# cswaney/NetworkHawkesProcesses.jl

Measured on AMD Instinct MI355X. Metric: log-likelihood evals/sec (N=1024, M=1e6), higher is better.
Workload: dtype f64; 1 GPU; continuous exponential standard Hawkes, N=1024, M=1000000, dt_max=1, windowed_k8 (S-metric, SURVEY 8d); pairs_per_eval=7999107, independent_streams=1

## Files before the change

networkhawkesprocesses.jl_amd/csrc/cont_slices.hip:

```cpp
#include <algorithm>
#include <vector>

#include "nhp_internal.h"
#include "nhp_math.h"
#include "nhp_rng.h"

struct nhp_slices {
    const uint32_t *row;
    const int32_t *item0;
    const uint32_t *lo;
    const uint16_t *hi;
    int32_t nsh;
    uint32_t dmask;
    int32_t dbits;
};

#define NHP_SL_SHARDS 64

#ifdef NHP_STAMP
__device__ unsigned long long g_sl_stamps[8 * 4096];
__device__ unsigned long long g_sl_wave_end[16 * 4096];
#define NHP_SL_STAMP(i) do { if (threadIdx.x == 0 && blockIdx.x < 4096) g_sl_stamps[8 * blockIdx.x + (i)] = __builtin_amdgcn_s_memrealtime(); } while (0)
#define NHP_SL_STAMP_WAVE() do { if ((threadIdx.x & 63) == 0 && blockIdx.x < 4096) g_sl_wave_end[16 * blockIdx.x + (threadIdx.x >> 6)] = __builtin_amdgcn_s_memrealtime(); } while (0)
extern "C" int nhp_debug_stamps_slices(unsigned long long *out, int n)
{
    return (int)hipMemcpyFromSymbol(out, HIP_SYMBOL(g_sl_stamps), sizeof(unsigned long long) * (size_t)n);
}
extern "C" int nhp_debug_stamps_slices_waves(unsigned long long *out, int n)
{
    return (int)hipMemcpyFromSymbol(out, HIP_SYMBOL(g_sl_wave_end), sizeof(unsigned long long) * (size_t)n);
}
#else
#define NHP_SL_STAMP(i) do { } while (0)
#define NHP_SL_STAMP_WAVE() do { } while (0)
#endif

extern "C" int32_t nhp_debug_slice_of(int32_t round, int32_t wave, int32_t nw) { return nhp_slice_of(round, wave, nw); }

__device__ __forceinline__ double sl_baseline(const nhp_cont_args &a, int c, double t)
{
#pragma clang fp contract(off)
    if (a.baseline_kind == NHP_BASELINE_HOMOGENEOUS) return a.lambda0[c];
    const double *x = a.grid;
    const double *y = a.lambda0 + (size_t)c * a.grid_n;
    int lo = 0, hi = a.grid_n - 1;
    if (!(t < x[hi])) return y[hi];
    while (hi - lo > 1) {
        const int mid = (lo + hi) >> 1;
        if (t >= x[mid]) lo = mid; else hi = mid;
    }
    return (y[lo + 1] * (t - x[lo]) + y[lo] * (x[lo + 1] - t)) / (x[lo + 1] - x[lo]);
}

__device__ __forceinline__ double sl_baseline_integral_col(const nhp_cont_args &a, int c)
{
    if (a.baseline_kind == NHP_BASELINE_HOMOGENEOUS) return threadIdx.x == 0 ? a.lambda0[c] * a.duration : 0.0;
    const double *y = a.lambda0 + (size_t)c * a.grid_n;
    double I = 0.0;
    for (int i = threadIdx.x; i + 1 < a.grid_n; i += blockDim.x) I += 0.5 * (y[i] + y[i + 1]) * (a.grid[i + 1] - a.grid[i]);
    return I;
}

__device__ __forceinline__ void sl_lgcp_scatter(const nhp_cont_args &a, int c, double t, double g, double *grad)
{
    const double *x = a.grid;
    const int G = a.grid_n;
    double *gc = grad + (size_t)c * G;
    int lo = 0, hi = G - 1;
    if (!(t < x[hi])) { atomicAdd(&gc[hi], g); return; }
    while (hi - lo > 1) {
        const int mid = (lo + hi) >> 1;
        if (t >= x[mid]) lo = mid; else hi = mid;
    }
    const double w = x[lo + 1] - x[lo];
    atomicAdd(&gc[lo], g * (x[lo + 1] - t) / w);
    atomicAdd(&gc[lo + 1], g * (t - x[lo]) / w);
}

__global__ __launch_bounds__(256) void k_slices_build(nhp_cont_args a, nhp_slices sl, uint32_t *__restrict__ lo, uint16_t *__restrict__ hi)
{
    const nhp_item it = a.items[blockIdx.x];
    const int lane = threadIdx.x & 63, w = threadIdx.x >> 6;
    const int nchild = it.kend - it.kbeg;
// ... 65 lines not shown
    for (int p = threadIdx.x; p < N; p += 256) {
        const uint32_t mine = c[p];
        int rank = 0;
        for (int q = 0; q < N; ++q) rank += (c[q] > mine || (c[q] == mine && q < p)) ? 1 : 0;
        perm[base + rank] = (uint16_t)p;
        rankof[(size_t)blockIdx.x * N + p] = (uint16_t)rank;
        if ((rank & 63) == 0) rows[(size_t)blockIdx.x * spi + (rank >> 6)] = mine;
    }
    for (int q = N + threadIdx.x; q < spi * 64; q += 256) perm[base + q] = 0xFFFFu;
}

__global__ __launch_bounds__(256) void k_ps_fill(nhp_cont_args a, nhp_pslices ps, const uint32_t *__restrict__ cnt, const uint16_t *__restrict__ rankof,
                                                 uint32_t *__restrict__ lo, uint16_t *__restrict__ hi)
{
    extern __shared__ __align__(16) unsigned char smem[];
    uint32_t *cursor = reinterpret_cast<uint32_t *>(smem);
    const nhp_item it = a.items[blockIdx.x];
    const int N = a.N;
    for (int p = threadIdx.x; p < N; p += 256) cursor[p] = 0;
    __syncthreads();
    const double two_d = __builtin_ldexp(1.0, ps.dbits);
    const double scale = a.inv_dtmax * two_d, qmax = two_d - 1.0;
    const uint32_t *row = ps.row + (size_t)blockIdx.x * ps.spi;
    for (int k = it.kbeg + threadIdx.x; k < it.kend; k += 256) {
        const nhp_child ch = a.child_w[k];
        const uint32_t slot = (uint32_t)(k - it.kbeg);
        for (int j = ch.idx - 1; j >= ch.first; --j) {
            const nhp_event e = a.ev[j];
            const uint32_t pos = atomicAdd(&cursor[e.node], 1u);
            const int rk = rankof[(size_t)blockIdx.x * N + e.node];
            double q = __builtin_rint((ch.t - e.t) * scale);
            q = q < 1.0 ? 1.0 : (q > qmax ? qmax : q);
            const uint64_t qi = (uint64_t)q;
            const size_t o = ((size_t)row[rk >> 6] + pos) * 64 + (size_t)(rk & 63);
            lo[o] = (uint32_t)qi;
            hi[o] = (uint16_t)((slot << ps.psh) | (uint32_t)(qi >> 32));
        }
    }
    for (int rk = threadIdx.x; rk < ps.spi * 64; rk += 256) {
        const int p = ps.perm[(size_t)blockIdx.x * ps.spi * 64 + rk];
        const uint32_t n = p == 0xFFFF ? 0u : cnt[(size_t)blockIdx.x * N + p];
        const uint32_t r0 = row[rk >> 6], R = row[(rk >> 6) + 1] - r0;
        for (uint32_t i = n; i < R; ++i) {
            const size_t o = ((size_t)r0 + i) * 64 + (size_t)(rk & 63);
            lo[o] = 0;
            hi[o] = (uint16_t)((uint32_t)ps.max_item << ps.psh);
        }
    }
}

__global__ __launch_bounds__(256) void k_ps_sort(int N, nhp_pslices ps, const uint32_t *__restrict__ cnt, uint32_t *__restrict__ lo,
                                                 uint16_t *__restrict__ hi)
{
    const uint32_t *row = ps.row + (size_t)blockIdx.x * ps.spi;
    for (int rk = threadIdx.x; rk < ps.spi * 64; rk += 256) {
        const int p = ps.perm[(size_t)blockIdx.x * ps.spi * 64 + rk];
        if (p == 0xFFFF) continue;
        const int n = (int)cnt[(size_t)blockIdx.x * N + p];
        const size_t o0 = (size_t)row[rk >> 6] * 64 + (size_t)(rk & 63);
        for (int i = 1; i < n; ++i) {
            const uint32_t l = lo[o0 + (size_t)i * 64], h = hi[o0 + (size_t)i * 64];
            const uint64_t key = ((uint64_t)h << 32) | l;
            int j = i - 1;
            while (j >= 0) {
                const uint32_t lj = lo[o0 + (size_t)j * 64], hj = hi[o0 + (size_t)j * 64];
                if ((((uint64_t)hj << 32) | lj) <= key) break;
                lo[o0 + (size_t)(j + 1) * 64] = lj;
                hi[o0 + (size_t)(j + 1) * 64] = (uint16_t)hj;
                --j;
            }
            lo[o0 + (size_t)(j + 1) * 64] = l;
            hi[o0 + (size_t)(j + 1) * 64] = (uint16_t)h;
        }
    }
}

__host__ __device__ constexpr size_t sl_exit_bytes(const int S, const int NW) { return ((size_t)S * NW * (17 * 8 + 17 * 8 + 17 * 4) + 15) / 16 * 16; }

static inline size_t sl_lds_bytes(const int N, const int S, const int block)
{
    return 320 + 16 * ((size_t)N + 1) * (size_t)S + 512 + sl_exit_bytes(S, block / 64);
}

__device__ __forceinline__ double sl_dpp_mul(const double v, const int sel)
{
#pragma clang fp contract(off)
    const int lo = __double2loint(v), hi = __double2hiint(v);
    int plo, phi;
    if (sel == 0) { plo = __builtin_amdgcn_mov_dpp(lo, 0xB1, 0xF, 0xF, true); phi = __builtin_amdgcn_mov_dpp(hi, 0xB1, 0xF, 0xF, true); }
    else { plo = __builtin_amdgcn_mov_dpp(lo, 0x4E, 0xF, 0xF, true); phi = __builtin_amdgcn_mov_dpp(hi, 0x4E, 0xF, 0xF, true); }
    return v * __hiloint2double(phi, plo);
}

template <int NW>
__device__ __forceinline__ void sl_exit_park(double v, double *__restrict__ park, const int m, const int w, const int lane)
{
#pragma clang fp contract(off)
    v = nhp_dpp_add(v, 0);
    v = nhp_dpp_add(v, 1);
    if ((lane & 3) == 0) park[(m * NW + w) * 17 + (lane >> 2)] = v;
}

template <int NW, int S>
__device__ __forceinline__ void sl_exit_sums(const double (&prod)[S], const int (&pexp)[S], double *__restrict__ park, double (&sx)[S], double (&sy)[S])
{
#pragma clang fp contract(off)
    constexpr int Q = S * NW;
    static_assert(Q <= 64, "one lane of the first wave per (model, wave)");
    double *qman = park + Q * 17;
    int *qexp = reinterpret_cast<int *>(qman + Q * 17);
    const int tid = threadIdx.x, lane = tid & 63;
    const int w = __builtin_amdgcn_readfirstlane(tid >> 6);
    double p[S];
    int e[S];
#pragma unroll
    for (int m = 0; m < S; ++m) {
        p[m] = sl_dpp_mul(sl_dpp_mul(prod[m], 0), 1);
        e[m] = pexp[m];
        e[m] += __builtin_amdgcn_mov_dpp(e[m], 0xB1, 0xF, 0xF, true);
        e[m] += __builtin_amdgcn_mov_dpp(e[m], 0x4E, 0xF, 0xF, true);
    }
    int ql = lane;
    asm volatile("" : "+v"(ql));
    if ((ql & 3) == 0) {
        const int o = w * 17 + (ql >> 2);
#pragma unroll
        for (int m = 0; m < S; ++m) {
            qman[m * NW * 17 + o] = p[m];
            qexp[m * NW * 17 + o] = e[m];
        }
    }
    __syncthreads();
    if (w != 0) return;
    if (lane < Q) {
        double *pm = qman + lane * 17;
        const int *pe = qexp + lane * 17;
        double *pk = park + lane * 17;
        double r = pm[0], si = 0.0;
        int es = pe[0];
#pragma unroll
        for (int i = 1; i < 16; ++i) r *= pm[i];
        asm volatile("" : "+v"(r) : : "memory");
#pragma unroll
        for (int i = 1; i < 16; ++i) es += pe[i];
        asm volatile("" : "+v"(es) : : "memory");
#pragma unroll
        for (int i = 0; i < 16; ++i) si += pk[i];
        asm volatile("" : "+v"(si) : : "memory");
        es += __builtin_amdgcn_frexp_exp(r);
        const double lg = nhp_log(__builtin_amdgcn_frexp_mant(r)) + (double)es * 6.93147180559945286e-01;
        pm[0] = lg;
        pk[0] = si;
    }
    __builtin_amdgcn_fence(__ATOMIC_RELEASE, "wavefront");
    __builtin_amdgcn_wave_barrier();
    __builtin_amdgcn_fence(__ATOMIC_ACQUIRE, "wavefront");
    if (tid == 0) {
#pragma unroll
        for (int m = 0; m < S; ++m) {
            double x = 0.0, y = 0.0;
            for (int q = 0; q < NW; ++q) { x += qman[(m * NW + q) * 17]; y += park[(m * NW + q) * 17]; }
            sx[m] = x; sy[m] = y;
        }
    }
}

template <int BLOCK, int C, bool FLAT, bool GRAD>
__global__ __launch_bounds__(BLOCK) void k_windowed_slices(nhp_cont_args a, nhp_slices sl, nhp_pslices ps, int mask_integral,
                                                            double *__restrict__ partials, unsigned int *__restrict__ counter,
                                                            double *__restrict__ out, int defer)
{
    constexpr int NW = BLOCK / 64;
    extern __shared__ __align__(16) unsigned char smem[];
    double *red = reinterpret_cast<double *>(smem);
    double2 *col = reinterpret_cast<double2 *>(smem + 320);
    double *etab = reinterpret_cast<double *>(col + a.N + 1);
    double *ginv = etab + 64;
    double *park = etab + 64;
    const int tid = threadIdx.x, lane = tid & 63;
    const double tab_v = nhp_exp2_64[lane];

    const nhp_item it = a.items[blockIdx.x];
    const int c = it.node, N = a.N;
    const int w = __builtin_amdgcn_readfirstlane(tid >> 6);
    const int nchild = it.kend - it.kbeg;
    const int s0 = sl.item0[blockIdx.x], ns = sl.item0[blockIdx.x + 1] - s0;
    NHP_SL_STAMP(0);

    struct chunk { uint32_t lo[C], hi[C]; };
    auto request = [&](chunk &q, const uint32_t *plo, const uint16_t *phi, const uint32_t row0, const int r) {
        const size_t o = ((size_t)row0 + (size_t)r) * 64;
        const uint32_t *pl = plo + o;
        const uint16_t *ph = phi + o;
#pragma unroll
        for (int u = 0; u < C; ++u) {
            q.lo[u] = pl[u * 64 + lane];
            q.hi[u] = ph[u * 64 + lane];
        }
    };
    constexpr int UN = BLOCK >= 512 ? 2 : 4;
    const double unit = __builtin_ldexp(a.dt_max, -sl.dbits);
    int j = w;
    uint32_t row0 = 0;
    int K = 0;
    chunk qa, qb;
    double integ = 0.0;
    for (int p0 = 0; p0 < N; p0 += UN * BLOCK) {
        double w_[UN], th_[UN], a_[UN], cnt_[UN];
#pragma unroll
        for (int u = 0; u < UN; ++u) {
            const int p = p0 + u * BLOCK + tid;
            const size_t k = (size_t)(p < N ? p : 0) + (size_t)c * N;
            w_[u] = a.W[k];
            th_[u] = a.p1[k];
            a_[u] = a.A ? a.A[k] : 1.0;
            cnt_[u] = it.first ? a.cnt[p < N ? p : 0] : 0.0;
        }
        if (p0 == 0) {
            if (j < ns) { row0 = sl.row[s0 + j]; K = (int)(sl.row[s0 + j + 1] - row0); }
            asm volatile("" ::: "memory");
            request(qa, sl.lo, sl.hi, row0, 0);
            asm volatile("" ::: "memory");
        }
#pragma unroll
        for (int u = 0; u < UN; ++u) {
            const int p = p0 + u * BLOCK + tid;
            if (p < N) {
                double wv = w_[u], wint = wv;
                if (a.A) {
                    wv = a_[u] * wv;
                    if (mask_integral) wint = wv;
                }
                col[p] = make_double2(-((th_[u] * unit) * 92.33248261689366), wv * th_[u]);
                integ += cnt_[u] * wint;
            }
        }
    }
    if (tid < 64) etab[tid] = tab_v;
    if (tid == 0) col[N] = make_double2(0.0, 0.0);
    if (GRAD && tid == 0) ginv[ps.max_item] = 0.0;
    if (out && it.first) integ += sl_baseline_integral_col(a, c);
    if (!GRAD) sl_exit_park<NW>(integ, park, 0, w, lane);
    __syncthreads();
    NHP_SL_STAMP(1);

    const double lam0 = FLAT ? a.lambda0[c] : 0.0;
    const uint32_t dmask = sl.dmask;
    const int nsh = sl.nsh;
    auto delay = [&](const uint32_t lo, const uint32_t h, const uint32_t mask) {
        uint32_t hw;
        asm("v_bfi_b32 %0, %1, %2, %3" : "=v"(hw) : "s"(mask), "v"(h), "v"(0x43300000u));
        return __hiloint2double((int)hw, (int)lo) - 4503599627370496.0;
    };
    auto term = [&](const uint32_t lo, const uint32_t h) {
        const double v = delay(lo, h, dmask);
        const double2 cw = col[h >> nsh];
        return cw.y * nhp_exp_neg_tab_scaled(cw.x * v, etab);
    };
    auto sum = [&](const chunk &q, const int r, const int K, double s) {
        if (r + C <= K) {
            double t[C];
#pragma unroll
            for (int u = 0; u < C; ++u) t[u] = term(q.lo[u], q.hi[u]);
#pragma unroll
            for (int u = 0; u < C; ++u) s += t[u];
        } else {
#pragma unroll
            for (int u = 0; u < C; ++u)
                if (r + u < K) s += term(q.lo[u], q.hi[u]);
        }
        return s;
    };
    double prod = 1.0, gsum = 0.0;
    int pexp = 0;
    int rnd = 0;
    while (j < ns) {
        const int jn = nhp_slice_of(++rnd, w, NW);
        uint32_t row0n = 0;
        int Kn = 0;
        if (jn < ns) { row0n = sl.row[s0 + jn]; Kn = (int)(sl.row[s0 + jn + 1] - row0n); }
        double s = 0.0;
        if (K <= 0) request(qa, sl.lo, sl.hi, row0n, 0);
        for (int r0 = 0; r0 < K; r0 += 2 * C) {
            request(qb, sl.lo, sl.hi, row0, r0 + C);
            asm volatile("" ::: "memory");
            s = sum(qa, r0, K, s);
            const bool more = r0 + 2 * C < K;
            request(qa, sl.lo, sl.hi, more ? row0 : row0n, more ? r0 + 2 * C : 0);
            asm volatile("" ::: "memory");
            s = sum(qb, r0 + C, K, s);
        }
        const int kk = 64 * j + lane;
        if (kk < nchild) {
            const double tk = FLAT ? 0.0 : a.child_w[it.kbeg + kk].t;
            const double lam = (FLAT ? lam0 : sl_baseline(a, c, tk)) + s;
            prod *= lam < 0.0 ? __builtin_nan("") : __builtin_amdgcn_frexp_mant(lam);
            pexp += __builtin_amdgcn_frexp_exp(lam);
            if (GRAD) {
                const double g = 1.0 / lam;
                ginv[kk] = g;
                if (FLAT) gsum += g;
                else sl_lgcp_scatter(a, c, tk, g, ps.grad);
            }
        }
        pexp += __builtin_amdgcn_frexp_exp(prod);
        prod = __builtin_amdgcn_frexp_mant(prod);
        j = jn; row0 = row0n; K = Kn;
    }
    NHP_SL_STAMP_WAVE();
    NHP_SL_STAMP(2);
    if (GRAD) {
        const uint32_t *prow = ps.row + (size_t)blockIdx.x * ps.spi;
        const uint16_t *pperm = ps.perm + (size_t)blockIdx.x * ps.spi * 64;
        const double punit = __builtin_ldexp(a.dt_max, -ps.dbits);
        const uint32_t pmask = ps.dmask;
        const int psh = ps.psh;
        const nhp_layout L(a);
        struct lanep { int p; double th, wv, av, cn; };
        auto lane_params = [&](const int jj) {
            lanep q;
            q.p = jj < ps.spi ? (int)pperm[jj * 64 + lane] : 0xFFFF;
            const size_t k = (size_t)(q.p == 0xFFFF ? 0 : q.p) + (size_t)c * N;
            q.th = a.p1[k];
            q.wv = a.W[k];
            q.av = a.A ? a.A[k] : 1.0;
            q.cn = ps.direct ? a.cnt[q.p == 0xFFFF ? 0 : q.p] : 0.0;
            return q;
        };
        int jp = w;
        uint32_t prow0 = 0;
        int Kp = 0;
        if (jp < ps.spi) { prow0 = prow[jp]; Kp = (int)(prow[jp + 1] - prow0); }
        lanep cur = lane_params(jp);
        request(qa, ps.lo, ps.hi, prow0, 0);
        __syncthreads();
        auto gterm = [&](const uint32_t lo, const uint32_t h, const double xs, double &accH, double &acc1) {
            const double v = delay(lo, h, pmask);
            const double g = ginv[h >> psh];
            const double t = xs * v;
            const double ge = g * nhp_exp_neg_tab_scaled(t, etab);
            accH += ge;
            acc1 = __builtin_fma(ge, __builtin_fma(t, 1.0830424696249145e-02, 1.0), acc1);
        };
        auto gsum_chunk = [&](const chunk &q, const int r, const int K, const double xs, double &accH, double &acc1) {
            if (r + C <= K) {
#pragma unroll
                for (int u = 0; u < C; ++u) gterm(q.lo[u], q.hi[u], xs, accH, acc1);
            } else {
#pragma unroll
                for (int u = 0; u < C; ++u)
                    if (r + u < K) gterm(q.lo[u], q.hi[u], xs, accH, acc1);
            }
        };
        while (jp < ps.spi) {
            const int jn = jp + NW;
            uint32_t row0n = 0;
            int Kn = 0;
            if (jn < ps.spi) { row0n = prow[jn]; Kn = (int)(prow[jn + 1] - row0n); }
            const lanep nxt = lane_params(jn);
            const double xs = -((cur.th * punit) * 92.33248261689366);
            double accH = 0.0, acc1 = 0.0;
            if (Kp <= 0) request(qa, ps.lo, ps.hi, row0n, 0);
            for (int r0 = 0; r0 < Kp; r0 += 2 * C) {
                request(qb, ps.lo, ps.hi, prow0, r0 + C);
                asm volatile("" ::: "memory");
                gsum_chunk(qa, r0, Kp, xs, accH, acc1);
                const bool more = r0 + 2 * C < Kp;
                request(qa, ps.lo, ps.hi, more ? prow0 : row0n, more ? r0 + 2 * C : 0);
                asm volatile("" ::: "memory");
                gsum_chunk(qb, r0 + C, Kp, xs, accH, acc1);
            }
            if (cur.p != 0xFFFF) {
                const size_t k = (size_t)cur.p + (size_t)c * N;
                const double gW = cur.av * (cur.th * accH);
// ... 43 lines not shown
    int *flag = reinterpret_cast<int *>(red + 32);
    if (tid == 0) {
        __hip_atomic_store(&partials[2 * (size_t)blockIdx.x], blk, __ATOMIC_RELAXED, __HIP_MEMORY_SCOPE_AGENT);
        __hip_atomic_store(&partials[2 * (size_t)blockIdx.x + 1], blk_int, __ATOMIC_RELAXED, __HIP_MEMORY_SCOPE_AGENT);
        asm volatile("s_waitcnt vmcnt(0)" ::: "memory");
        const unsigned int nb = gridDim.x, sh = blockIdx.x % NHP_SL_SHARDS;
        const unsigned int pop = (nb - sh + NHP_SL_SHARDS - 1) / NHP_SL_SHARDS;
        const unsigned int used = nb < NHP_SL_SHARDS ? nb : NHP_SL_SHARDS;
        int last = 0;
        if (__hip_atomic_fetch_add(&counter[32 * (1 + sh)], 1u, __ATOMIC_RELAXED, __HIP_MEMORY_SCOPE_AGENT) == pop - 1)
            last = __hip_atomic_fetch_add(&counter[0], 1u, __ATOMIC_RELAXED, __HIP_MEMORY_SCOPE_AGENT) == used - 1;
        *flag = last;
    }
    __syncthreads();
    NHP_SL_STAMP(4);
    if (!*flag) return;
    double sl_ = 0.0, si = 0.0;
    for (unsigned int i = tid; i < gridDim.x; i += BLOCK) {
        sl_ += __hip_atomic_load(&partials[2 * (size_t)i], __ATOMIC_RELAXED, __HIP_MEMORY_SCOPE_AGENT);
        si += __hip_atomic_load(&partials[2 * (size_t)i + 1], __ATOMIC_RELAXED, __HIP_MEMORY_SCOPE_AGENT);
    }
    nhp_block_sum2_n<NW>(sl_, si, red);
    if (tid == 0) *out = (0.0 - si) + sl_;
    for (int i = tid; i <= NHP_SL_SHARDS; i += BLOCK)
        __hip_atomic_store(&counter[32 * i], 0u, __ATOMIC_RELAXED, __HIP_MEMORY_SCOPE_AGENT);
}

#define NHP_SETS_MAX 4
struct nhp_sets {
    const double *p1[NHP_SETS_MAX], *W[NHP_SETS_MAX], *A[NHP_SETS_MAX], *lambda0[NHP_SETS_MAX];
    double *out[NHP_SETS_MAX];
};

__device__ __forceinline__ double sl_flat_integral(const double lam0, const double duration)
{
#pragma clang fp contract(off)
    return threadIdx.x == 0 ? lam0 * duration : 0.0;
}

template <int BLOCK, int C, int S, bool DEFER = false>
__global__ __launch_bounds__(BLOCK) void k_slices_batch(nhp_cont_args a, nhp_slices sl, nhp_sets st, double *__restrict__ partials,
                                                         unsigned int *__restrict__ counter)
{
    constexpr int NW = BLOCK / 64;
    extern __shared__ __align__(16) unsigned char smem[];
    double *red = reinterpret_cast<double *>(smem);
    double2 *col = reinterpret_cast<double2 *>(smem + 320);
    double *etab = reinterpret_cast<double *>(col + (size_t)S * (a.N + 1));
    double *park = etab + 64;
    const int tid = threadIdx.x, lane = tid & 63;
    const double tab_v = nhp_exp2_64[lane];
    const nhp_item it = a.items[blockIdx.x];
    const int c = it.node, N = a.N;
    const int w = __builtin_amdgcn_readfirstlane(tid >> 6);
    const int nchild = it.kend - it.kbeg;
    const int s0 = sl.item0[blockIdx.x], ns = sl.item0[blockIdx.x + 1] - s0;
    NHP_SL_STAMP(0);

    struct chunk { uint32_t lo[C], hi[C]; };
    auto request = [&](chunk &q, const uint32_t row0, const int r) {
        const size_t o = ((size_t)row0 + (size_t)r) * 64;
        const uint32_t *pl = sl.lo + o;
        const uint16_t *ph = sl.hi + o;
#pragma unroll
        for (int u = 0; u < C; ++u) {
            q.lo[u] = pl[u * 64 + lane];
            q.hi[u] = ph[u * 64 + lane];
        }
    };
    constexpr int UN = 2;
    constexpr int G = S >= 2 ? 2 : 1;
    const size_t c0 = (size_t)c * N;
    typedef const __attribute__((address_space(1))) double *gptr;
    gptr Wc[S], Tc[S], Ac[S];
    double lam0[S];
#pragma unroll
    for (int m = 0; m < S; ++m) {
        Wc[m] = (gptr)st.W[m]; Tc[m] = (gptr)st.p1[m]; Ac[m] = (gptr)st.A[m];
        lam0[m] = st.lambda0[m][c];
    }
#pragma unroll
    for (int m = 0; m < S; ++m) asm("" : "+s"(Wc[m]), "+s"(Tc[m]), "+s"(Ac[m]));
    const double unit = __builtin_ldexp(a.dt_max, -sl.dbits);
    int j = w;
    uint32_t row0 = 0;
    int K = 0;
    chunk qa, qb;
    double integ[S];
#pragma unroll
    for (int m = 0; m < S; ++m) integ[m] = 0.0;
    const bool first = DEFER ? true : it.first != 0;
    gptr cntp = (gptr)a.cnt;
    auto at = [](gptr base, const uint32_t off) {
        return *(gptr)((const __attribute__((address_space(1))) char *)base + off);
    };
    for (int p0 = 0; p0 < N; p0 += UN * BLOCK) {
        double cnt_[UN];
        uint32_t off_[UN];
#pragma unroll
        for (int u = 0; u < UN; ++u) {
            const int p = p0 + u * BLOCK + tid;
            off_[u] = (uint32_t)(p < N ? p : 0) * 8u;
            cnt_[u] = first ? at(cntp, off_[u]) : 0.0;
        }
#pragma unroll
        for (int g = 0; g < S; g += G) {
            double w_[G][UN], th_[G][UN], a_[G][UN], wv_[G][UN];
#pragma unroll
            for (int mm = 0; mm < G; ++mm) {
                const int m = g + mm;
#pragma unroll
                for (int u = 0; u < UN; ++u) {
                    w_[mm][u] = at(Wc[m] + c0, off_[u]);
                    th_[mm][u] = at(Tc[m] + c0, off_[u]);
                    a_[mm][u] = Ac[m] ? at(Ac[m] + c0, off_[u]) : 1.0;
                }
            }
            if (p0 == 0 && g == 0) {
                if (j < ns) { row0 = sl.row[s0 + j]; K = (int)(sl.row[s0 + j + 1] - row0); }
                asm volatile("" ::: "memory");
                request(qa, row0, 0);
                asm volatile("" ::: "memory");
            }
#pragma unroll
            for (int mm = 0; mm < G; ++mm) {
                const int m = g + mm;
#pragma unroll
                for (int u = 0; u < UN; ++u) {
                    const int p = p0 + u * BLOCK + tid;
                    wv_[mm][u] = a_[mm][u] * w_[mm][u];
                    if (p < N) {
                        col[(size_t)m * (N + 1) + p] = make_double2(-((th_[mm][u] * unit) * 92.33248261689366), wv_[mm][u] * th_[mm][u]);
                        if (DEFER) integ[m] += cnt_[u] * wv_[mm][u];
                    }
                }
            }
            if (!DEFER && first) {
#pragma unroll
                for (int mm = 0; mm < G; ++mm)
#pragma unroll
                    for (int u = 0; u < UN; ++u)
                        if (p0 + u * BLOCK + tid < N) integ[g + mm] += cnt_[u] * wv_[mm][u];
            }
        }
    }
#pragma unroll
    for (int m = 0; m < S; ++m) {
        if (tid == 0) col[(size_t)m * (N + 1) + N] = make_double2(0.0, 0.0);
        if (first) integ[m] += sl_flat_integral(lam0[m], a.duration);
        sl_exit_park<NW>(integ[m], park, m, w, lane);
    }
    if (tid < 64) etab[tid] = tab_v;
    __syncthreads();
    NHP_SL_STAMP(1);

    const uint32_t dmask = sl.dmask;
    const int nsh = sl.nsh;
    const uint32_t plane = (uint32_t)(N + 1) * 16u;
    auto terms = [&](const uint32_t lo, const uint32_t h, double (&acc)[S]) {
        uint32_t hw;
        asm("v_bfi_b32 %0, %1, %2, %3" : "=v"(hw) : "s"(dmask), "v"(h), "v"(0x43300000u));
        const double v = __hiloint2double((int)hw, (int)lo) - 4503599627370496.0;
        const unsigned char *base = reinterpret_cast<const unsigned char *>(col) + ((h >> nsh) << 4);
#pragma unroll
        for (int m = 0; m < S; ++m) {
            const double2 cw = *reinterpret_cast<const double2 *>(base + m * plane);
            acc[m] = __builtin_fma(cw.y, nhp_exp_neg_tab_scaled(cw.x * v, etab), acc[m]);
        }
    };
    auto sum = [&](const chunk &q, const int r, const int K, double (&acc)[S]) {
        if (r + C <= K) {
#pragma unroll
            for (int u = 0; u < C; ++u) terms(q.lo[u], q.hi[u], acc);
        } else {
#pragma unroll
            for (int u = 0; u < C; ++u)
                if (r + u < K) terms(q.lo[u], q.hi[u], acc);
        }
    };
    double prod[S];
    int pexp[S];
#pragma unroll
    for (int m = 0; m < S; ++m) { prod[m] = 1.0; pexp[m] = 0; }
    int rnd = 0;
    while (j < ns) {
        const int jn = nhp_slice_of(++rnd, w, NW);
        uint32_t row0n = 0;
        int Kn = 0;
        if (jn < ns) { row0n = sl.row[s0 + jn]; Kn = (int)(sl.row[s0 + jn + 1] - row0n); }
        double acc[S];
#pragma unroll
        for (int m = 0; m < S; ++m) acc[m] = 0.0;
        if (K <= 0) request(qa, row0n, 0);
        for (int r0 = 0; r0 < K; r0 += 2 * C) {
            request(qb, row0, r0 + C);
            asm volatile("" ::: "memory");
            sum(qa, r0, K, acc);
            const bool more = r0 + 2 * C < K;
            request(qa, more ? row0 : row0n, more ? r0 + 2 * C : 0);
            asm volatile("" ::: "memory");
            sum(qb, r0 + C, K, acc);
        }
        const int kk = 64 * j + lane;
        if (kk < nchild) {
#pragma unroll
            for (int m = 0; m < S; ++m) {
                const double lam = lam0[m] + acc[m];
                prod[m] *= lam < 0.0 ? __builtin_nan("") : __builtin_amdgcn_frexp_mant(lam);
                pexp[m] += __builtin_amdgcn_frexp_exp(lam);
            }
        }
#pragma unroll
        for (int m = 0; m < S; ++m) {
            pexp[m] += __builtin_amdgcn_frexp_exp(prod[m]);
            prod[m] = __builtin_amdgcn_frexp_mant(prod[m]);
        }
        j = jn; row0 = row0n; K = Kn;
    }
    NHP_SL_STAMP_WAVE();
    NHP_SL_STAMP(2);
    double sx[S], sy[S];
#pragma unroll
    for (int m = 0; m < S; ++m) { sx[m] = 0.0; sy[m] = 0.0; }
    sl_exit_sums<NW, S>(prod, pexp, park, sx, sy);
    NHP_SL_STAMP(3);
    if (DEFER) {
        if (tid == 0) {
#pragma unroll
            for (int m = 0; m < S; ++m) {
                st.out[m][2 * (size_t)blockIdx.x] = sx[m];
                st.out[m][2 * (size_t)blockIdx.x + 1] = sy[m];
            }
        }
        NHP_SL_STAMP(4);
        return;
    }
    int *flag = reinterpret_cast<int *>(red + 32);
    if (tid == 0) {
#pragma unroll
        for (int m = 0; m < S; ++m) {
            __hip_atomic_store(&partials[(2 * (size_t)blockIdx.x) * S + 2 * m], sx[m], __ATOMIC_RELAXED, __HIP_MEMORY_SCOPE_AGENT);
            __hip_atomic_store(&partials[(2 * (size_t)blockIdx.x) * S + 2 * m + 1], sy[m], __ATOMIC_RELAXED, __HIP_MEMORY_SCOPE_AGENT);
        }
        asm volatile("s_waitcnt vmcnt(0)" ::: "memory");
        const unsigned int nb = gridDim.x, sh = blockIdx.x % NHP_SL_SHARDS;
        const unsigned int pop = (nb - sh + NHP_SL_SHARDS - 1) / NHP_SL_SHARDS;
        const unsigned int used = nb < NHP_SL_SHARDS ? nb : NHP_SL_SHARDS;
        int last = 0;
        if (__hip_atomic_fetch_add(&counter[32 * (1 + sh)], 1u, __ATOMIC_RELAXED, __HIP_MEMORY_SCOPE_AGENT) == pop - 1)
            last = __hip_atomic_fetch_add(&counter[0], 1u, __ATOMIC_RELAXED, __HIP_MEMORY_SCOPE_AGENT) == used - 1;
        *flag = last;
    }
    __syncthreads();
    NHP_SL_STAMP(4);
    if (!*flag) return;
#pragma unroll
    for (int m = 0; m < S; ++m) {
        double sl_ = 0.0, si = 0.0;
        for (unsigned int i = tid; i < gridDim.x; i += BLOCK) {
            sl_ += __hip_atomic_load(&partials[(2 * (size_t)i) * S + 2 * m], __ATOMIC_RELAXED, __HIP_MEMORY_SCOPE_AGENT);
            si += __hip_atomic_load(&partials[(2 * (size_t)i) * S + 2 * m + 1], __ATOMIC_RELAXED, __HIP_MEMORY_SCOPE_AGENT);
        }
        nhp_block_sum2_n<NW>(sl_, si, red);
        if (tid == 0) *st.out[m] = (0.0 - si) + sl_;
        __syncthreads();
    }
    for (int i = tid; i <= NHP_SL_SHARDS; i += BLOCK)
        __hip_atomic_store(&counter[32 * i], 0u, __ATOMIC_RELAXED, __HIP_MEMORY_SCOPE_AGENT);
}

__global__ __launch_bounds__(256) void k_slices_build_lq(nhp_cont_args a, nhp_slices sl, double *__restrict__ L, double *__restrict__ Q)
{
#pragma clang fp contract(off)
    const nhp_item it = a.items[blockIdx.x];
    const int lane = threadIdx.x & 63, w = threadIdx.x >> 6;
    const int nchild = it.kend - it.kbeg;
    const int s0 = sl.item0[blockIdx.x], ns = sl.item0[blockIdx.x + 1] - s0;
    for (int j = w; j < ns; j += 4) {
        const uint32_t row0 = sl.row[s0 + j];
        const int K = (int)(sl.row[s0 + j + 1] - row0);
        const int kk = 64 * j + lane;
        nhp_child ch;
        ch.t = 0.0; ch.first = 0; ch.idx = 0;
        if (kk < nchild) ch = a.child_w[it.kbeg + kk];
        const int len = ch.idx - ch.first;
        for (int r = 0; r < K; ++r) {
            double2 d = make_double2(0.0, 0.0);
            if (r < len) d = nhp_logitnormal_data(a.inv_dtmax, ch.t - a.ev[ch.idx - 1 - r].t);
            const size_t o = ((size_t)row0 + (size_t)r) * 64 + (size_t)lane;
            L[o] = d.x;
            Q[o] = d.y;
        }
    }
}

__global__ __launch_bounds__(256) void k_slices_build_d(nhp_cont_args a, nhp_slices sl, double *__restrict__ D)
{
    const nhp_item it = a.items[blockIdx.x];
    const int lane = threadIdx.x & 63, w = threadIdx.x >> 6;
    const int nchild = it.kend - it.kbeg;
    const int s0 = sl.item0[blockIdx.x], ns = sl.item0[blockIdx.x + 1] - s0;
// ... 696 lines not shown
```

networkhawkesprocesses.jl_amd/csrc/nhp_math.h:

```cpp
#pragma once
#include <hip/hip_runtime.h>
#include <stdint.h>

#define NHP_INVSQRT2PI 0.3989422804014327

__device__ __forceinline__ double nhp_horner(double p, double r, double c)
{
    double d;
    asm("v_fma_f64 %0, %1, %2, %3" : "=v"(d) : "v"(p), "v"(r), "s"(c));
    return d;
}

__device__ __forceinline__ double nhp_horner13(double r)
{
    double p;
    const double c13 = 1.6059043836821613e-10;
    asm("v_fma_f64 %0, %1, %2, %3\n\t"
        "v_fma_f64 %0, %0, %2, %4\n\t"
        "v_fma_f64 %0, %0, %2, %5\n\t"
        "v_fma_f64 %0, %0, %2, %6\n\t"
        "v_fma_f64 %0, %0, %2, %7\n\t"
        "v_fma_f64 %0, %0, %2, %8\n\t"
        "v_fma_f64 %0, %0, %2, %9\n\t"
        "v_fma_f64 %0, %0, %2, %10\n\t"
// ... 34 lines not shown
    double r = __builtin_fma(-n, LN2_HI, x);
    r = __builtin_fma(-n, LN2_LO, r);
    double p = nhp_horner13(r);
    double v = __builtin_ldexp(p, (int)n);
    return (x >= -708.0) ? v : 0.0;
}

__device__ __forceinline__ double nhp_exp_neg_ll(double x)
{
#pragma clang fp contract(off)
    const double LOG2E = 1.44269504088896338700e+00;
    const double LN2_HI = 6.93147180369123816490e-01;
    const double LN2_LO = 1.90821492927058770002e-10;
    double n = __builtin_rint(x * LOG2E);
    double r = __builtin_fma(-n, LN2_HI, x);
    r = __builtin_fma(-n, LN2_LO, r);
    return __builtin_ldexp(nhp_horner13(r), (int)n);
}

static __device__ const double nhp_exp2_64[64] = {
    0x1.0000000000000p+0, 0x1.02c9a3e778061p+0, 0x1.059b0d3158574p+0, 0x1.0874518759bc8p+0,
    0x1.0b5586cf9890fp+0, 0x1.0e3ec32d3d1a2p+0, 0x1.11301d0125b51p+0, 0x1.1429aaea92de0p+0,
    0x1.172b83c7d517bp+0, 0x1.1a35beb6fcb75p+0, 0x1.1d4873168b9aap+0, 0x1.2063b88628cd6p+0,
    0x1.2387a6e756238p+0, 0x1.26b4565e27cddp+0, 0x1.29e9df51fdee1p+0, 0x1.2d285a6e4030bp+0,
    0x1.306fe0a31b715p+0, 0x1.33c08b26416ffp+0, 0x1.371a7373aa9cbp+0, 0x1.3a7db34e59ff7p+0,
    0x1.3dea64c123422p+0, 0x1.4160a21f72e2ap+0, 0x1.44e086061892dp+0, 0x1.486a2b5c13cd0p+0,
    0x1.4bfdad5362a27p+0, 0x1.4f9b2769d2ca7p+0, 0x1.5342b569d4f82p+0, 0x1.56f4736b527dap+0,
    0x1.5ab07dd485429p+0, 0x1.5e76f15ad2148p+0, 0x1.6247eb03a5585p+0, 0x1.6623882552225p+0,
    0x1.6a09e667f3bcdp+0, 0x1.6dfb23c651a2fp+0, 0x1.71f75e8ec5f74p+0, 0x1.75feb564267c9p+0,
    0x1.7a11473eb0187p+0, 0x1.7e2f336cf4e62p+0, 0x1.82589994cce13p+0, 0x1.868d99b4492edp+0,
    0x1.8ace5422aa0dbp+0, 0x1.8f1ae99157736p+0, 0x1.93737b0cdc5e5p+0, 0x1.97d829fde4e50p+0,
    0x1.9c49182a3f090p+0, 0x1.a0c667b5de565p+0, 0x1.a5503b23e255dp+0, 0x1.a9e6b5579fdbfp+0,
    0x1.ae89f995ad3adp+0, 0x1.b33a2b84f15fbp+0, 0x1.b7f76f2fb5e47p+0, 0x1.bcc1e904bc1d2p+0,
    0x1.c199bdd85529cp+0, 0x1.c67f12e57d14bp+0, 0x1.cb720dcef9069p+0, 0x1.d072d4a07897cp+0,
    0x1.d5818dcfba487p+0, 0x1.da9e603db3285p+0, 0x1.dfc97337b9b5fp+0, 0x1.e502ee78b3ff6p+0,
    0x1.ea4afa2a490dap+0, 0x1.efa1bee615a27p+0, 0x1.f50765b6e4540p+0, 0x1.fa7c1819e90d8p+0,
};

__device__ __forceinline__ void nhp_exp_tab_init(double *tab)
{
    if (threadIdx.x < 64) tab[threadIdx.x] = nhp_exp2_64[threadIdx.x];
}

__device__ __forceinline__ double nhp_exp_neg_tab(double x, const double *tab)
{
#pragma clang fp contract(off)
    const double K64 = 92.33248261689366;
    const double L64_HI = 0x1.62e42ff000000p-7;
    const double L64_LO = -0x1.718432a1b0e26p-41;
    const double kf = __builtin_rint(x * K64);
    double r = __builtin_fma(-kf, L64_HI, x);
    r = __builtin_fma(-kf, L64_LO, r);
    const int k = (int)kf;
    const double t = tab[k & 63];
    double p;
    const double c5 = 8.3333333333333332e-03;
    asm("v_fma_f64 %0, %1, %2, %3\n\t"
        "v_fma_f64 %0, %0, %2, %4\n\t"
        "v_fma_f64 %0, %0, %2, 0.5\n\t"
        "v_fma_f64 %0, %0, %2, 1.0\n\t"
        "v_mul_f64 %0, %0, %2"
        : "=&v"(p)
        : "v"(c5), "v"(r), "s"(4.1666666666666664e-02), "s"(1.6666666666666666e-01));
    return __builtin_ldexp(__builtin_fma(t, p, t), k >> 6);
}

__device__ __forceinline__ double nhp_exp_neg_tab_scaled(double t, const double *tab)
{
#pragma clang fp contract(off)
    const double kf = __builtin_rint(t);
    const double u = t - kf;
    const int k = (int)kf;
    const double tb = tab[k & 63];
    double p;
    const double c5 = 0x1.5d87fe78a6731p-40;
    asm("v_fma_f64 %0, %1, %2, %3\n\t"
        "v_fma_f64 %0, %0, %2, %4\n\t"
        "v_fma_f64 %0, %0, %2, %5\n\t"
        "v_fma_f64 %0, %0, %2, %6\n\t"
        "v_mul_f64 %0, %0, %2"
        : "=&v"(p)
        : "v"(c5), "v"(u), "s"(0x1.3b2ab6fba4e77p-31), "s"(0x1.c6b08d704a0c0p-23), "s"(0x1.ebfbdff82c58fp-15), "s"(0x1.62e42fefa39efp-7));
    return __builtin_ldexp(__builtin_fma(tb, p, tb), k >> 6);
}

__device__ __forceinline__ double nhp_pdf_exponential_tab(double r, double dt, const double *tab)
{
#pragma clang fp contract(off)
    return r * nhp_exp_neg_tab(-(r * dt), tab);
}

__device__ __forceinline__ double nhp_log(double x)
{
#pragma clang fp contract(off)
    const double ln2_hi = 6.93147180369123816490e-01;
    const double ln2_lo = 1.90821492927058770002e-10;
    const double Lg1 = 6.666666666666735130e-01, Lg2 = 3.999999999940941908e-01,
                 Lg3 = 2.857142874366239149e-01, Lg4 = 2.222219843214978396e-01,
                 Lg5 = 1.818357216161805012e-01, Lg6 = 1.531383769920937332e-01,
                 Lg7 = 1.479819860511658591e-01;
    uint64_t u = (uint64_t)__double_as_longlong(x);
    uint32_t hx = (uint32_t)(u >> 32);
    int k = 0;
    if (hx < 0x00100000u || (hx >> 31)) {
        if ((u << 1) == 0) return -__builtin_inf();
        if (hx >> 31) return __builtin_nan("");
        k -= 54;
        x *= 18014398509481984.0;
        u = (uint64_t)__double_as_longlong(x);
        hx = (uint32_t)(u >> 32);
    } else if (hx >= 0x7ff00000u) {
        return x;
    } else if (hx == 0x3ff00000u && (u << 32) == 0) {
        return 0.0;
    }
    hx += 0x3ff00000u - 0x3fe6a09eu;
    k += (int)(hx >> 20) - 0x3ff;
    hx = (hx & 0x000fffffu) + 0x3fe6a09eu;
    u = ((uint64_t)hx << 32) | (u & 0xffffffffu);
    x = __longlong_as_double((long long)u);
    double f = x - 1.0;
    double hfsq = 0.5 * f * f;
    double s = f / (2.0 + f);
    double z = s * s;
    double w = z * z;
    double t1 = w * (Lg2 + w * (Lg4 + w * Lg6));
    double t2 = z * (Lg1 + w * (Lg3 + w * (Lg5 + w * Lg7)));
    double R = t2 + t1;
    double dk = (double)k;
    return s * (hfsq + R) + dk * ln2_lo - hfsq + f + dk * ln2_hi;
}

__host__ __device__ __forceinline__ double nhp_philox_uniform(uint64_t seed, uint64_t step, uint64_t event)
{
    uint32_t c0 = (uint32_t)event, c1 = (uint32_t)(event >> 32);
    uint32_t c2 = (uint32_t)step, c3 = (uint32_t)(step >> 32);
    uint32_t k0 = (uint32_t)seed, k1 = (uint32_t)(seed >> 32);
    for (int r = 0; r < 10; ++r) {
        uint64_t p0 = (uint64_t)0xD2511F53u * c0;
        uint64_t p1 = (uint64_t)0xCD9E8D57u * c2;
        uint32_t n0 = (uint32_t)(p1 >> 32) ^ c1 ^ k0;
        uint32_t n1 = (uint32_t)p1;
        uint32_t n2 = (uint32_t)(p0 >> 32) ^ c3 ^ k1;
        uint32_t n3 = (uint32_t)p0;
        c0 = n0; c1 = n1; c2 = n2; c3 = n3;
        k0 += 0x9E3779B9u; k1 += 0xBB67AE85u;
    }
    uint64_t bits = ((uint64_t)c0 << 32) | c1;
    return (double)(bits >> 11) * 1.1102230246251565e-16;
}


__device__ __forceinline__ double nhp_pdf_exponential(double r, double dt)
{
#pragma clang fp contract(off)
    return r * nhp_exp_neg(-(r * dt));
}

__device__ __forceinline__ double nhp_pdf_exponential_ll(double r, double dt)
{
#pragma clang fp contract(off)
#ifdef NHP_EXP_STUB
    return r * (1.0 - 1e-3 * (r * dt));
#else
    return r * nhp_exp_neg_ll(-(r * dt));
#endif
// ... 32 lines not shown
```

Measured before the change: 120,300 log-likelihood evals/sec.

## Use magic-number rounding and exponent-bit scaling for exp terms when range allows

```diff
diff --git a/networkhawkesprocesses.jl_amd/csrc/cont_slices.hip b/networkhawkesprocesses.jl_amd/csrc/cont_slices.hip
--- a/networkhawkesprocesses.jl_amd/csrc/cont_slices.hip
+++ b/networkhawkesprocesses.jl_amd/csrc/cont_slices.hip
@@ -1,4 +1,5 @@
 #include <algorithm>
+#include <type_traits>
 #include <vector>
 
 #include "nhp_internal.h"
@@ -230,6 +231,19 @@
     return 320 + 16 * ((size_t)N + 1) * (size_t)S + 512 + sl_exit_bytes(S, block / 64);
 }
 
+__device__ __forceinline__ double sl_term_limit(const int dbits) { return __builtin_ldexp(NHP_EXP_TERM_LIMIT, -dbits); }
+__device__ __forceinline__ bool sl_term_outside(const double cx, const double lim) { return !(__builtin_fabs(cx) <= lim); }
+__device__ __forceinline__ void sl_limit_post(const bool bad, int *__restrict__ flg, const int w, const int lane)
+{
+    const bool any = __builtin_amdgcn_ballot_w64(bad) != 0;
+    if (lane == 0) flg[w] = any ? 1 : 0;
+}
+template <int NW>
+__device__ __forceinline__ bool sl_limit_all_inside(const int *__restrict__ flg, const int lane)
+{
+    return __builtin_amdgcn_ballot_w64(flg[lane & (NW - 1)] != 0) == 0;
+}
+
 __device__ __forceinline__ double sl_dpp_mul(const double v, const int sel)
 {
 #pragma clang fp contract(off)
@@ -348,6 +362,8 @@
     };
     constexpr int UN = BLOCK >= 512 ? 2 : 4;
     const double unit = __builtin_ldexp(a.dt_max, -sl.dbits);
+    const double tlim = GRAD ? 0.0 : sl_term_limit(sl.dbits);
+    bool outside = false;
     int j = w;
     uint32_t row0 = 0;
     int K = 0;
@@ -380,45 +396,65 @@
                     if (mask_integral) wint = wv;
                 }
                 col[p] = make_double2(-((th_[u] * unit) * 92.33248261689366), wv * th_[u]);
+                if constexpr (!GRAD) outside |= sl_term_outside(-((th_[u] * unit) * 92.33248261689366), tlim);
                 integ += cnt_[u] * wint;
             }
         }
     }
-    if (tid < 64) etab[tid] = tab_v;
+    if (tid < 64) etab[tid] = GRAD ? tab_v : nhp_exp_tab_biased(tab_v, tid);
     if (tid == 0) col[N] = make_double2(0.0, 0.0);
     if (GRAD && tid == 0) ginv[ps.max_item] = 0.0;
     if (out && it.first) integ += sl_baseline_integral_col(a, c);
-    if (!GRAD) sl_exit_park<NW>(integ, park, 0, w, lane);
+    if constexpr (!GRAD) {
+        sl_exit_park<NW>(integ, park, 0, w, lane);
+        sl_limit_post(outside, reinterpret_cast<int *>(red), w, lane);
+    }
     __syncthreads();
     NHP_SL_STAMP(1);
+    const bool fast = GRAD ? false : sl_limit_all_inside<NW>(reinterpret_cast<const int *>(red), lane);
 
     const double lam0 = FLAT ? a.lambda0[c] : 0.0;
     const uint32_t dmask = sl.dmask;
     const int nsh = sl.nsh;
+    const nhp_exp_term_consts ekc = nhp_exp_term_setup();
     auto delay = [&](const uint32_t lo, const uint32_t h, const uint32_t mask) {
         uint32_t hw;
         asm("v_bfi_b32 %0, %1, %2, %3" : "=v"(hw) : "s"(mask), "v"(h), "v"(0x43300000u));
         return __hiloint2double((int)hw, (int)lo) - 4503599627370496.0;
     };
-    auto term = [&](const uint32_t lo, const uint32_t h) {
+    auto term = [&](auto mode, const uint32_t lo, const uint32_t h) {
+        constexpr int MODE = decltype(mode)::value;
         const double v = delay(lo, h, dmask);
         const double2 cw = col[h >> nsh];
-        return cw.y * nhp_exp_neg_tab_scaled(cw.x * v, etab);
+        if constexpr (MODE == 0) return cw.y * nhp_exp_neg_tab_scaled(cw.x * v, etab);
+        else if constexpr (MODE == 1) return cw.y * nhp_exp_term_fast(cw.x, v, etab, ekc);
+        else return cw.y * nhp_exp_term_slow(cw.x, v, etab, ekc);
     };
-    auto sum = [&](const chunk &q, const int r, const int K, double s) {
-        if (r + C <= K) {
+    auto sum = [&](auto mode, const chunk &q, const int r, const int K, double s) {
+        constexpr int MODE = decltype(mode)::value;
+        if (MODE != 2 && r + C <= K) {
             double t[C];
 #pragma unroll
-            for (int u = 0; u < C; ++u) t[u] = term(q.lo[u], q.hi[u]);
+            for (int u = 0; u < C; ++u) t[u] = term(mode, q.lo[u], q.hi[u]);
 #pragma unroll
             for (int u = 0; u < C; ++u) s += t[u];
         } else {
 #pragma unroll
             for (int u = 0; u < C; ++u)
-                if (r + u < K) s += term(q.lo[u], q.hi[u]);
+                if (r + u < K) s += term(mode, q.lo[u], q.hi[u]);
         }
         return s;
     };
+#define NHP_SL_ROWS(mode)                                                                                             \
+    for (int r0 = 0; r0 < K; r0 += 2 * C) {                                                                           \
+        request(qb, sl.lo, sl.hi, row0, r0 + C);                                                                      \
+        asm volatile("" ::: "memory");                                                                                \
+        s = sum(mode, qa, r0, K, s);                                                                                  \
+        const bool more = r0 + 2 * C < K;                                                                             \
+        request(qa, sl.lo, sl.hi, more ? row0 : row0n, more ? r0 + 2 * C : 0);                                        \
+        asm volatile("" ::: "memory");                                                                                \
+        s = sum(mode, qb, r0 + C, K, s);                                                                              \
+    }
     double prod = 1.0, gsum = 0.0;
     int pexp = 0;
     int rnd = 0;
@@ -429,15 +465,10 @@
         if (jn < ns) { row0n = sl.row[s0 + jn]; Kn = (int)(sl.row[s0 + jn + 1] - row0n); }
         double s = 0.0;
         if (K <= 0) request(qa, sl.lo, sl.hi, row0n, 0);
-        for (int r0 = 0; r0 < K; r0 += 2 * C) {
-            request(qb, sl.lo, sl.hi, row0, r0 + C);
-            asm volatile("" ::: "memory");
-            s = sum(qa, r0, K, s);
-            const bool more = r0 + 2 * C < K;
-            request(qa, sl.lo, sl.hi, more ? row0 : row0n, more ? r0 + 2 * C : 0);
-            asm volatile("" ::: "memory");
-            s = sum(qb, r0 + C, K, s);
-        }
+        if constexpr (GRAD) { NHP_SL_ROWS((std::integral_constant<int, 0>{})) }
+        else if (fast) { NHP_SL_ROWS((std::integral_constant<int, 1>{})) }
+        else { NHP_SL_ROWS((std::integral_constant<int, 2>{})) }
+#undef NHP_SL_ROWS
         const int kk = 64 * j + lane;
         if (kk < nchild) {
             const double tk = FLAT ? 0.0 : a.child_w[it.kbeg + kk].t;
@@ -647,6 +678,8 @@
 #pragma unroll
     for (int m = 0; m < S; ++m) asm("" : "+s"(Wc[m]), "+s"(Tc[m]), "+s"(Ac[m]));
     const double unit = __builtin_ldexp(a.dt_max, -sl.dbits);
+    const double tlim = sl_term_limit(sl.dbits);
+    bool outside = false;
     int j = w;
     uint32_t row0 = 0;
     int K = 0;
@@ -695,7 +728,9 @@
                     const int p = p0 + u * BLOCK + tid;
                     wv_[mm][u] = a_[mm][u] * w_[mm][u];
                     if (p < N) {
-                        col[(size_t)m * (N + 1) + p] = make_double2(-((th_[mm][u] * unit) * 92.33248261689366), wv_[mm][u] * th_[mm][u]);
+                        const double cx = -((th_[mm][u] * unit) * 92.33248261689366);
+                        col[(size_t)m * (N + 1) + p] = make_double2(cx, wv_[mm][u] * th_[mm][u]);
+                        outside |= sl_term_outside(cx, tlim);
                         if (DEFER) integ[m] += cnt_[u] * wv_[mm][u];
                     }
                 }
@@ -715,73 +750,81 @@
         if (first) integ[m] += sl_flat_integral(lam0[m], a.duration);
         sl_exit_park<NW>(integ[m], park, m, w, lane);
     }
-    if (tid < 64) etab[tid] = tab_v;
+    if (tid < 64) etab[tid] = nhp_exp_tab_biased(tab_v, tid);
+    sl_limit_post(outside, reinterpret_cast<int *>(red), w, lane);
     __syncthreads();
     NHP_SL_STAMP(1);
+    const bool fast = sl_limit_all_inside<NW>(reinterpret_cast<const int *>(red), lane);
 
     const uint32_t dmask = sl.dmask;
     const int nsh = sl.nsh;
+    const nhp_exp_term_consts ekc = nhp_exp_term_setup();
     const uint32_t plane = (uint32_t)(N + 1) * 16u;
-    auto terms = [&](const uint32_t lo, const uint32_t h, double (&acc)[S]) {
-        uint32_t hw;
-        asm("v_bfi_b32 %0, %1, %2, %3" : "=v"(hw) : "s"(dmask), "v"(h), "v"(0x43300000u));
-        const double v = __hiloint2double((int)hw, (int)lo) - 4503599627370496.0;
-        const unsigned char *base = reinterpret_cast<const unsigned char *>(col) + ((h >> nsh) << 4);
-#pragma unroll
-        for (int m = 0; m < S; ++m) {
-            const double2 cw = *reinterpret_cast<const double2 *>(base + m * plane);
-            acc[m] = __builtin_fma(cw.y, nhp_exp_neg_tab_scaled(cw.x * v, etab), acc[m]);
-        }
-    };
-    auto sum = [&](const chunk &q, const int r, const int K, double (&acc)[S]) {
-        if (r + C <= K) {
-#pragma unroll
-            for (int u = 0; u < C; ++u) terms(q.lo[u], q.hi[u], acc);
-        } else {
-#pragma unroll
-            for (int u = 0; u < C; ++u)
-                if (r + u < K) terms(q.lo[u], q.hi[u], acc);
-        }
-    };
     double prod[S];
     int pexp[S];
 #pragma unroll
     for (int m = 0; m < S; ++m) { prod[m] = 1.0; pexp[m] = 0; }
     int rnd = 0;
-    while (j < ns) {
-        const int jn = nhp_slice_of(++rnd, w, NW);
-        uint32_t row0n = 0;
-        int Kn = 0;
-        if (jn < ns) { row0n = sl.row[s0 + jn]; Kn = (int)(sl.row[s0 + jn + 1] - row0n); }
-        double acc[S];
-#pragma unroll
-        for (int m = 0; m < S; ++m) acc[m] = 0.0;
-        if (K <= 0) request(qa, row0n, 0);
-        for (int r0 = 0; r0 < K; r0 += 2 * C) {
-            request(qb, row0, r0 + C);
-            asm volatile("" ::: "memory");
-            sum(qa, r0, K, acc);
-            const bool more = r0 + 2 * C < K;
-            request(qa, more ? row0 : row0n, more ? r0 + 2 * C : 0);
-            asm volatile("" ::: "memory");
-            sum(qb, r0 + C, K, acc);
-        }
-        const int kk = 64 * j + lane;
-        if (kk < nchild) {
+    auto walk = [&](auto fastc) {
+        constexpr bool FAST = decltype(fastc)::value;
+        auto terms = [&](const uint32_t lo, const uint32_t h, double (&acc)[S]) {
+            uint32_t hw;
+            asm("v_bfi_b32 %0, %1, %2, %3" : "=v"(hw) : "s"(dmask), "v"(h), "v"(0x43300000u));
+            const double v = __hiloint2double((int)hw, (int)lo) - 4503599627370496.0;
+            const unsigned char *base = reinterpret_cast<const unsigned char *>(col) + ((h >> nsh) << 4);
 #pragma unroll
             for (int m = 0; m < S; ++m) {
-                const double lam = lam0[m] + acc[m];
-                prod[m] *= lam < 0.0 ? __builtin_nan("") : __builtin_amdgcn_frexp_mant(lam);
-                pexp[m] += __builtin_amdgcn_frexp_exp(lam);
-            }
-        }
-#pragma unroll
-        for (int m = 0; m < S; ++m) {
-            pexp[m] += __builtin_amdgcn_frexp_exp(prod[m]);
-            prod[m] = __builtin_amdgcn_frexp_mant(prod[m]);
-        }
-        j = jn; row0 = row0n; K = Kn;
-    }
+                const double2 cw = *reinterpret_cast<const double2 *>(base + m * plane);
+                if constexpr (FAST) acc[m] = __builtin_fma(cw.y, nhp_exp_term_fast(cw.x, v, etab, ekc), acc[m]);
+                else acc[m] = __builtin_fma(cw.y, nhp_exp_term_slow(cw.x, v, etab, ekc), acc[m]);
+            }
+        };
+        auto sum = [&](const chunk &q, const int r, const int K, double (&acc)[S]) {
+            if (FAST && r + C <= K) {
+#pragma unroll
+                for (int u = 0; u < C; ++u) terms(q.lo[u], q.hi[u], acc);
+            } else {
+#pragma unroll
+                for (int u = 0; u < C; ++u)
+                    if (r + u < K) terms(q.lo[u], q.hi[u], acc);
+            }
+        };
+        while (j < ns) {
+            const int jn = nhp_slice_of(++rnd, w, NW);
+            uint32_t row0n = 0;
+            int Kn = 0;
+            if (jn < ns) { row0n = sl.row[s0 + jn]; Kn = (int)(sl.row[s0 + jn + 1] - row0n); }
+            double acc[S];
+#pragma unroll
+            for (int m = 0; m < S; ++m) acc[m] = 0.0;
+            if (K <= 0) request(qa, row0n, 0);
+            for (int r0 = 0; r0 < K; r0 += 2 * C) {
+                request(qb, row0, r0 + C);
+                asm volatile("" ::: "memory");
+                sum(qa, r0, K, acc);
+                const bool more = r0 + 2 * C < K;
+                request(qa, more ? row0 : row0n, more ? r0 + 2 * C : 0);
+                asm volatile("" ::: "memory");
+                sum(qb, r0 + C, K, acc);
+            }
+            const int kk = 64 * j + lane;
+            if (kk < nchild) {
+#pragma unroll
+                for (int m = 0; m < S; ++m) {
+                    const double lam = lam0[m] + acc[m];
+                    prod[m] *= lam < 0.0 ? __builtin_nan("") : __builtin_amdgcn_frexp_mant(lam);
+                    pexp[m] += __builtin_amdgcn_frexp_exp(lam);
+                }
+            }
+#pragma unroll
+            for (int m = 0; m < S; ++m) {
+                pexp[m] += __builtin_amdgcn_frexp_exp(prod[m]);
+                prod[m] = __builtin_amdgcn_frexp_mant(prod[m]);
+            }
+            j = jn; row0 = row0n; K = Kn;
+        }
+    };
+    if (fast) walk(std::true_type{}); else walk(std::false_type{});
     NHP_SL_STAMP_WAVE();
     NHP_SL_STAMP(2);
     double sx[S], sy[S];
diff --git a/networkhawkesprocesses.jl_amd/csrc/nhp_math.h b/networkhawkesprocesses.jl_amd/csrc/nhp_math.h
--- a/networkhawkesprocesses.jl_amd/csrc/nhp_math.h
+++ b/networkhawkesprocesses.jl_amd/csrc/nhp_math.h
@@ -140,6 +140,64 @@
         : "=&v"(p)
         : "v"(c5), "v"(u), "s"(0x1.3b2ab6fba4e77p-31), "s"(0x1.c6b08d704a0c0p-23), "s"(0x1.ebfbdff82c58fp-15), "s"(0x1.62e42fefa39efp-7));
     return __builtin_ldexp(__builtin_fma(tb, p, tb), k >> 6);
+}
+
+#define NHP_EXP_TERM_MAGIC 6755399441055744.0
+#define NHP_EXP_TERM_LIMIT 65000.0
+
+__device__ __forceinline__ double nhp_exp_tab_biased(const double e, const int j)
+{
+    return __hiloint2double((int)((uint32_t)__double2hiint(e) - ((uint32_t)j << 14)), __double2loint(e));
+}
+
+struct nhp_exp_term_consts { double magic, top; };
+__device__ __forceinline__ nhp_exp_term_consts nhp_exp_term_setup()
+{
+    nhp_exp_term_consts c;
+    c.magic = NHP_EXP_TERM_MAGIC;
+    c.top = 0x1.5d87fe78a6731p-40;
+    asm("" : "+s"(c.magic));
+    asm("" : "+v"(c.top));
+    return c;
+}
+
+__device__ __forceinline__ double nhp_exp_term_poly(const double u, const double top)
+{
+    double p;
+    asm("v_fma_f64 %0, %1, %2, %3\n\t"
+        "v_fma_f64 %0, %0, %2, %4\n\t"
+        "v_fma_f64 %0, %0, %2, %5\n\t"
+        "v_fma_f64 %0, %0, %2, %6\n\t"
+        "v_mul_f64 %0, %0, %2"
+        : "=&v"(p)
+        : "v"(top), "v"(u), "s"(0x1.3b2ab6fba4e77p-31), "s"(0x1.c6b08d704a0c0p-23), "s"(0x1.ebfbdff82c58fp-15), "s"(0x1.62e42fefa39efp-7));
+    return p;
+}
+
+__device__ __forceinline__ double nhp_exp_term_fast(const double cx, const double v, const double *tabb, const nhp_exp_term_consts &kc)
+{
+#pragma clang fp contract(off)
+    const double km = __builtin_fma(cx, v, kc.magic);
+    const double kf = km - kc.magic;
+    const double u = __builtin_fma(cx, v, -kf);
+    const uint32_t k = (uint32_t)__double2loint(km);
+    const double tb = tabb[k & 63u];
+    const double ts = __hiloint2double((int)((k << 14) + (uint32_t)__double2hiint(tb)), __double2loint(tb));
+    return __builtin_fma(ts, nhp_exp_term_poly(u, kc.top), ts);
+}
+
+__device__ __forceinline__ double nhp_exp_term_slow(const double cx, const double v, const double *tabb, const nhp_exp_term_consts &kc)
+{
+#pragma clang fp contract(off)
+    const double km = __builtin_fma(cx, v, kc.magic);
+    const double kf = km - kc.magic;
+    const double u = __builtin_fma(cx, v, -kf);
+    const int k = (int)kf;
+    const double us = (__builtin_fabs(kf) >= 0x1p31 && __builtin_fabs(kf) < __builtin_inf()) ? 0.0 : u;
+    const uint32_t j = (uint32_t)k & 63u;
+    const double tb = tabb[j];
+    const double t1 = __hiloint2double((int)((j << 14) + (uint32_t)__double2hiint(tb)), __double2loint(tb));
+    return __builtin_ldexp(__builtin_fma(t1, nhp_exp_term_poly(us, kc.top), t1), k >> 6);
 }
 
 __device__ __forceinline__ double nhp_pdf_exponential_tab(double r, double dt, const double *tab)
```

Result: faster. 123,500 log-likelihood evals/sec (median of 6 runs) (+2.6%).
